# AndreeaPatarlageanu/ConcurrentProject

Hardware: AMD Instinct MI355X
Metric: GCUPS (cell updates/s) for NxN affine-gap SW; bit-exact score vs CPU (higher is better)
Workload: dtype int32; 1 GPU; C2 single pair N=65536 (seed 65536); N=65536, pairs_per_gpu=1, global_pairs=1, parallelism=single GPU, kernel_items=262, blocks=256, boundary_bytes=263207296, W=2, kernel=flow3, half-chunk links, kernel_fn=sw_flow3_kernel, C=32, step=linear-gap identity (G_INIT == G_EXT, exact)

## Files before the change

### concurrentproject_amd/csrc/sw_engine.hip

```cpp
#include "sw_internal.h"
#include "../../include/algoGPU.h"

#include <rccl/rccl.h>
#include <dlfcn.h>

#include <algorithm>
#include <atomic>
#include <chrono>
#include <condition_variable>
#include <functional>
#include <thread>
#include <cstdarg>
#include <cstdio>
#include <cstdlib>
#include <cstring>
#include <map>
#include <mutex>
#include <set>
#include <string>
#include <vector>

namespace swmi {
namespace {

// ... 82 lines not shown
    X(duo_tab, 1, 0, 2, nullptr, false)                                                                               \
                                              \
    X(duo_roles, 1, 0, 1, nullptr, false)                                                                             \
                                         \
    X(duo_raw, 1, 0, 1, nullptr, false)                                                                               \
        \
    X(duo_prio, -1, -1, 20, opt_prio_ok, false)                                                                       \
                                                   \
    X(slab_plain, 0, 0, 1, nullptr, false)                                                                            \
                                                    \
    X(stall_item, -1, -1, ANY_HI, nullptr, false)

#define X(key, def, lo, hi, ok, flag) O_##key,
enum Opt : int { SW_OPTIONS(X) OPT_COUNT };
#undef X
struct OptRow {
    const char* key;
    long long def, lo, hi;
    bool (*ok)(long long);
    bool flag;
};
#define X(key, def, lo, hi, ok, flag) {#key, def, lo, hi, ok, flag},
constexpr OptRow OPT_ROWS[OPT_COUNT] = {SW_OPTIONS(X)};
#undef X
#define X(key, def, lo, hi, ok, flag) {def},
std::atomic<long long> g_opt[OPT_COUNT] = {SW_OPTIONS(X)};
#undef X

struct Opts {
    long long v[OPT_COUNT];
    int f3wedge = -1;
    int f3drops_set = 0;
    int f3drops[4] = {64, 64, 64, 64};
    long long operator[](Opt o) const { return v[o]; }
};
Opts snapshot_opts() {
    Opts o;
    for (int i = 0; i < OPT_COUNT; ++i) o.v[i] = g_opt[i].load();
    const char* w = std::getenv("SWMI_F3WEDGE");
    o.f3wedge = w && w[0] == '0' && !w[1] ? 0 : w && w[0] == '1' && !w[1] ? 1 : -1;
    if (const char* d = std::getenv("SWMI_F3WEDGE_DROPS")) {
        char tail = 0;
        const int got = std::sscanf(d, "%d,%d,%d,%d%c", &o.f3drops[0], &o.f3drops[1], &o.f3drops[2], &o.f3drops[3], &tail);
        o.f3drops_set = got == 4 && wedge_drops_ok(o.f3drops) ? 1 : -1;
    }
    return o;
}
int find_opt(const char* key) {
    for (int i = 0; i < OPT_COUNT; ++i)
        if (std::strcmp(key, OPT_ROWS[i].key) == 0) return i;
    return -1;
}

constexpr long long MAX_SEQ = (1LL << 27) - 1;
constexpr long long RING_AUTO_BYTES = 1LL << 30;

bool want_swap(const Opts& opt, bool single, long long len1, long long len2) {
    const long long o = opt[O_orient];
    if (o == 1) return false;
    if (o == 2) return true;
    return single ? (len2 > len1) : (len1 > len2);
}

bool params_ok(const Params& p) {
    if (p.gap_init < 0 || p.gap_ext < 0 || p.gap_init > (1 << 20) || p.gap_ext > (1 << 20)) {
        set_err("unsupported gap penalties (%d, %d): need 0 <= G_INIT, G_EXT <= 2^20", p.gap_init, p.gap_ext);
        return false;
    }
    if (p.mismatch > 0 || p.mismatch < -127 || p.match > 127 || p.match < p.mismatch) {
        set_err("unsupported scores (MATCH %d, MISMATCH %d): need -127 <= MISMATCH <= 0, MISMATCH <= MATCH <= 127",
                p.match, p.mismatch);
        return false;
    }
// ... 29 lines not shown
        if (p) { HIPCHK(hipHostFree(p)); p = nullptr; cap = 0; }
        size_t want = std::max<size_t>(n, 1);
        want = want + want / 4;
        HIPCHK(hipHostMalloc((void**)&p, want * sizeof(T), hipHostMallocDefault));
        cap = want;
        return 0;
    }
};

struct Ctx {
    int dev = -1;
    int cus = 256;
    hipStream_t own = nullptr;
    hipStream_t last = nullptr;
    hipEvent_t ev0 = nullptr, ev1 = nullptr, staged = nullptr;
    bool staged_pending = false;
    DevBuf<unsigned char> seq;
    DevBuf<PairDesc> desc;
    DevBuf<int> ibase;
    DevBuf<Granule> bnd;
    DevBuf<Ctrl> ctrl;
    DevBuf<int> scores;
    DevBuf<unsigned> flag;
    DevBuf<unsigned> cons;
    DevBuf<unsigned char> hrows;
    DevBuf<DuoDesc> duo;
    PinBuf<DuoDesc> hduo;
    PinBuf<unsigned char> hseq;
    PinBuf<PairDesc> hdesc;
    PinBuf<int> hibase;
    PinBuf<int> hscores;
    PinBuf<Ctrl> hctrl;
    unsigned epoch = 0;
    std::map<int, int> waves_cache;
};

thread_local std::map<int, Ctx*> t_ctx;

Ctx* get_ctx() {
    int dev = 0;
    if (hipGetDevice(&dev) != hipSuccess) {
        set_err("hipGetDevice failed: no HIP device");
        return nullptr;
    }
    auto it = t_ctx.find(dev);
    if (it != t_ctx.end()) return it->second;
    Ctx* c = new Ctx();
    c->dev = dev;
    hipDeviceProp_t prop;
    if (hipGetDeviceProperties(&prop, dev) != hipSuccess) {
        set_err("hipGetDeviceProperties failed");
        delete c;
        return nullptr;
    }
    c->cus = prop.multiProcessorCount;
    if (hipStreamCreateWithFlags(&c->own, hipStreamNonBlocking) != hipSuccess ||
        hipEventCreate(&c->ev0) != hipSuccess || hipEventCreate(&c->ev1) != hipSuccess ||
        hipEventCreateWithFlags(&c->staged, hipEventDisableTiming) != hipSuccess) {
        set_err("stream/event creation failed");
        delete c;
        return nullptr;
    }
    t_ctx[dev] = c;
    return c;
}

// ... 675 lines not shown
    }
    g.wrap_rows = 1;
    while (g.wrap_rows < job.pairs[0].m) g.wrap_rows *= 2;
    job.bnd_granules = (uint64_t)(g.blocks - 1) * (uint64_t)opt[O_ring_rows] + (uint64_t)g.wrap_rows;
    return 0;
}

int size_grid(Ctx* c, Job& job, Variant& v, const Opts& opt, size_t np, Grid& g) {
    const int items = job.item_base[np];
    g.f2_wgs = pick_f2_wgs(job, v, opt, c->cus, items);
    if (v.cfg.duo_wrap > 0) job.bnd_granules = 0;
    if (v.ring && size_ring(job, v, opt, c->cus, items, g)) return -1;
    v.cfg.f2_wgs = g.f2_wgs;
    g.wpc = waves_per_cu(c, v.cfg);
    long long blocks = opt[O_blocks];
    if (blocks <= 0) {
        const int wpb = job.mode == MODE_DUO ? DUO_WAVES : 4;
        const long long cap = (long long)c->cus * std::max(1, g.wpc / wpb);
        const long long want = job.mode == MODE_STRIP ? (items + 3) / 4 : grouped_mode(job.mode) ? items : (long long)np;
        blocks = std::min<long long>(want, cap);
        if (job.mode == MODE_FLOW2) blocks = std::min<long long>(blocks, (long long)c->cus * g.f2_wgs);
    }
    if (v.ring) blocks = g.blocks;
    if (job.f3pwg) {
        blocks = std::min<long long>(np, opt[O_blocks] > 0 ? opt[O_blocks] : (long long)c->cus * g.f2_wgs);
        g.wrap_rows = 64;
        while (g.wrap_rows < v.cfg.max_m) g.wrap_rows *= 2;
        job.bnd_granules = (uint64_t)blocks * (uint64_t)g.wrap_rows;
    }
    v.cfg.blocks = g.blocks = (int)std::max<long long>(1, blocks);
    return 0;
}

int stage_descriptors(Ctx* c, const Job& job, size_t np, hipStream_t s) {
    const bool duo = job.mode == MODE_DUO;
    if (c->staged_pending) {
        HIPCHK(hipEventSynchronize(c->staged));
        c->staged_pending = false;
    }
    if (c->hdesc.ensure(np) || c->hibase.ensure(np + 1) || c->hduo.ensure(np)) return -1;
    if (duo) std::memcpy(c->hduo.p, job.duos.data(), np * sizeof(DuoDesc));
    else std::memcpy(c->hdesc.p, job.pairs.data(), np * sizeof(PairDesc));
    std::memcpy(c->hibase.p, job.item_base.data(), (np + 1) * sizeof(int));
    const Ctrl* ctrl_before = c->ctrl.p;
    if (c->desc.ensure(np, s) || c->duo.ensure(np, s) || c->ibase.ensure(np + 1, s) || c->ctrl.ensure(1, s)) return -1;
    if (c->ctrl.p != ctrl_before) HIPCHK(hipMemsetAsync(c->ctrl.p, 0, sizeof(Ctrl), s));
    return 0;
}

int prepare_device(Ctx* c, const Job& job, const Variant& v, const Opts& opt, const unsigned char* d_seq, int* d_scores,
                   int nscores, size_t np, hipStream_t s) {
    const size_t cons = v.ring ? (size_t)v.cfg.blocks * RING_CONS_STRIDE
                        : v.cfg.duo_wrap > 0 && opt[O_duo_roles] != 0 ? (size_t)DUO_CU_WORDS : 0;
    if (cons) {
        if (c->cons.ensure(cons, s)) return -1;
        HIPCHK(hipMemsetAsync(c->cons.p, 0, cons * sizeof(unsigned), s));
    }
    if (job.bnd_granules) {
        size_t freeb = 0, totb = 0;
        HIPCHK(hipMemGetInfo(&freeb, &totb));
        const size_t need = job.bnd_granules * sizeof(Granule);
        if (need > c->bnd.cap * sizeof(Granule) && need > freeb / 10 * 9) {
            set_err("strip-boundary buffers need %.2f GB, %.2f GB free", need / 1e9, freeb / 1e9);
            return -1;
        }
        if (c->bnd.ensure(job.bnd_granules, s)) return -1;
    }
    if (job.mode == MODE_DUO) HIPCHK(hipMemcpyAsync(c->duo.p, c->hduo.p, np * sizeof(DuoDesc), hipMemcpyHostToDevice, s));
    else HIPCHK(hipMemcpyAsync(c->desc.p, c->hdesc.p, np * sizeof(PairDesc), hipMemcpyHostToDevice, s));
    HIPCHK(hipMemcpyAsync(c->ibase.p, c->hibase.p, (np + 1) * sizeof(int), hipMemcpyHostToDevice, s));
    HIPCHK(hipEventRecord(c->staged, s));
    c->staged_pending = true;
    HIPCHK(hipMemsetAsync(c->ctrl.p, 0, sizeof(unsigned), s));
    HIPCHK(hipMemsetAsync(d_scores, 0, (size_t)nscores * sizeof(int), s));
    if (v.cfg.hep && v.ring) {
        const PairDesc& d = job.pairs[0];
        if (c->hrows.ensure((size_t)d.m, s)) return -1;
        HepSel t{};
        for (int b = 0; b < 256; ++b) {
            const unsigned sym = job.hsym[b];
            t.sel[b] = (unsigned char)(sym < 4 ? 4 + sym : sym - 3);
        }
        hipLaunchKernelGGL(hep_rows_kernel, dim3((unsigned)std::min(1024, (d.m + 255) / 256)), dim3(256), 0, s,
                           d_seq + d.row_off, d.m, c->hrows.p, t);
        HIPCHK(hipGetLastError());
    }
    return 0;
}

void fill_score_words(KParams& kp, const Params& prm, const unsigned char* hsym) {
    kp.match = prm.match;
    kp.mismatch = prm.mismatch;
    kp.gap_init = prm.gap_init;
    kp.gap_ext = prm.gap_ext;
    profile_words(prm, kp.prof);
    for (int q = 0; q < 4; ++q) {
        unsigned w2 = 0, w3 = 0, pen = 0;
        for (int r = 0; r < 4; ++r) {
            const int sc = r == q ? prm.match : prm.mismatch;
            w2 |= (unsigned)((sc + prm.gap_init) & 0xFF) << (8 * r);
            w3 |= (unsigned)(sc & 0xFF) << (8 * r);
            pen |= (unsigned)(prm.match - sc) << (8 * r);
        }
        kp.prof2[q] = w2;
        kp.prof3[q] = w3;
        kp.pen[q] = pen;
    }
    if (!hsym) return;
    std::memcpy(kp.hsym, hsym, sizeof kp.hsym);
    for (int c = 0; c < 7; ++c) {
        unsigned p2 = 0, q2 = 0x80u, p3 = 0, q3 = 0x80u;
        for (int r = 0; r < 7; ++r) {
            const int sc = r == c ? prm.match : prm.mismatch;
            const unsigned b2 = (unsigned)((sc + prm.gap_init) & 0xFF), b3 = (unsigned)(sc & 0xFF);
            if (r < 4) {
                p2 |= b2 << (8 * r);
                p3 |= b3 << (8 * r);
            } else {
                q2 |= b2 << (8 * (r - 3));
                q3 |= b3 << (8 * (r - 3));
            }
        }
        kp.hp2[c] = p2;
        kp.hq2[c] = q2;
        kp.hp3[c] = p3;
        kp.hq3[c] = q3;
    }
}

KParams fill_kparams(Ctx* c, const Job& job, const Variant& v, const Grid& g, const Params& prm, const Opts& opt,
                     const unsigned char* d_seq, int* d_scores, size_t np, const SlabEdge* edge) {
    KParams kp{};
    kp.seq = d_seq;
    kp.pairs = c->desc.p;
    kp.duos = c->duo.p;
    kp.item_base = c->ibase.p;
    kp.bnd = c->bnd.p;
    kp.ctrl = c->ctrl.p;
    kp.scores = d_scores;
    kp.npairs = (int)np;
    kp.total_items = job.item_base[np];
    do ++c->epoch;
    while (c->epoch == 0 || ((c->epoch ^ 0x5BD1E995u) & 31u) == 0 || ((c->epoch ^ 0x5BD1E995u ^ 0x9E3779B9u) & 31u) == 0);
    kp.epoch = c->epoch;
    fill_score_words(kp, prm, v.cfg.hep ? job.hsym : nullptr);
    if (v.cfg.duo_wrap > 0) {
        kp.wrap_rows = v.cfg.duo_wrap;
        if (opt[O_duo_roles] != 0) kp.ring_cons = c->cons.p;
        const int dp = (int)opt[O_duo_prio];
        kp.duo_prio = dp >= 0 ? dp : v.cfg.duo_tab > 0 ? 17 : 0;
    }
    kp.timeout_ticks = opt[O_timeout] * 100000000LL;
    kp.stall_item = (int)opt[O_stall_item];
    kp.w45_s4 = v.cfg.f3_w45 ? job.w45_s4 : -1;
    kp.trace = reinterpret_cast<unsigned long long*>(opt[O_trace]);
    if (v.ring) {
        kp.ring_rows = (int)opt[O_ring_rows];
        kp.wrap_rows = g.wrap_rows;
        kp.ring_cons = c->cons.p;
    }
    if (job.f3pwg) kp.wrap_rows = g.wrap_rows;
    if (v.wedge) {
        kp.wedge = 1;
        kp.wedge_e0[0] = job.wplan.e0[0];
        kp.wedge_e0[1] = job.wplan.e0[1];
        kp.wedge_rlead = job.wplan.rlead;
        kp.wedge_rows = job.wedge_rows;
        kp.wedge_bnd[0] = job.wedge_bnd[0];
        kp.wedge_bnd[1] = job.wedge_bnd[1];
        for (int j = 0; j < 4; ++j) kp.wedge_drop[j] = job.wplan.drop[j];
        kp.wedge_segr = job.wedge_segr;
        kp.wedge_seg[0] = job.wedge_seg[0];
        kp.wedge_seg[1] = job.wedge_seg[1];
    }
    if (v.cfg.hep && v.ring) kp.hrows = c->hrows.p;
    if (edge) {
        kp.slab_in = edge->in;
        kp.slab_out = edge->out;
        kp.slab_epoch = edge->epoch;
    }
    return kp;
}

int enqueue(Ctx* c, Job& job, const Params& prm, const Opts& opt, const unsigned char* d_seq, int* d_scores, int nscores,
            hipStream_t s, bool time_kernel, const SlabEdge* edge = nullptr) {
    if (job.mode == MODE_FLOW2 ? !flow2_variant_exists(job.C) : !variant_exists(job.W, job.C)) {
        set_err("no kernel variant for W=%d C=%d", job.W, job.C);
        return -1;
    }
    if (opt.f3drops_set < 0) {
        set_err("SWMI_F3WEDGE_DROPS: need d0,d1,d2,d3, multiples of 64 from 64 to %d with d0 == d2", WEDGE_DROP_MAX);
        return -1;
    }
    if (!plan_wedge(job, prm, opt, c->cus)) plan_split(job, prm, opt, c->cus);
    Variant v = select_variant(job, prm, opt, c->cus);
    if (v.err) {
        set_err("%s", v.err);
        return -1;
    }
    const size_t np = job.mode == MODE_DUO ? job.duos.size() : job.pairs.size();
    Grid g;
    if (stage_descriptors(c, job, np, s) || size_grid(c, job, v, opt, np, g) ||
        prepare_device(c, job, v, opt, d_seq, d_scores, nscores, np, s))
        return -1;
    const KParams kp = fill_kparams(c, job, v, g, prm, opt, d_seq, d_scores, np, edge);

    if (time_kernel) HIPCHK(hipEventRecord(c->ev0, s));
    HIPCHK(v.cfg.f3 || v.cfg.f3a || v.cfg.f3ra ? launch_sw_flow3(v.cfg, kp, s)
           : job.mode == MODE_FLOW2           ? launch_sw_flow2(v.cfg, kp, s) : launch_sw_strip(v.cfg, kp, s));
    if (v.cut) {
        const PairDesc& l = job.pairs[0];
        const PairDesc& r = job.pairs[1];
        const Granule* gl = c->bnd.p + l.bnd_off + (uint64_t)((l.strips + 3) / 4 - 1) * (uint64_t)l.m;
        const Granule* gr = c->bnd.p + r.bnd_off + (uint64_t)((r.strips + 3) / 4 - 1) * (uint64_t)r.m;
        HIPCHK(launch_sw_flow3_combine(gl, gr, l.m, prm.gap_init, kp.epoch, c->ctrl.p, d_scores + l.out_idx, s));
    }
    if (v.steep) {
        const SteepJoin j = {c->bnd.p + job.wedge_bnd[0], c->bnd.p + job.wedge_bnd[1], c->bnd.p + job.pairs[0].bnd_off,
                             c->bnd.p + job.pairs[1].bnd_off, c->bnd.p + job.wedge_seg[0], c->bnd.p + job.wedge_seg[1],
                             job.wedge_rows, job.wedge_segr, job.pairs[0].m, prm.gap_init};
        HIPCHK(launch_sw_flow3_steep_combine(j, job.wplan, kp.epoch, c->ctrl.p, d_scores + job.pairs[0].out_idx, s));
    } else if (v.wedge)
        HIPCHK(launch_sw_flow3_wedge_combine(c->bnd.p + job.wedge_bnd[0], c->bnd.p + job.wedge_bnd[1], job.wplan,
                                             job.pairs[0].m, kp.epoch, c->ctrl.p, d_scores + job.pairs[0].out_idx, s));
    if (time_kernel) HIPCHK(hipEventRecord(c->ev1, s));

    t_stats = sw_stats{};
    t_stats.cells = job.cells;
    t_stats.W = job.W;
    t_stats.C = job.C;
    t_stats.dna = job.hep ? 2 : job.dna ? 1 : 0;
    t_stats.blocks = v.cfg.blocks;
    t_stats.waves_per_cu = g.wpc;
    t_stats.items = job.item_base[np];
    t_stats.mode = job.mode;
    t_stats.variant = variant_word(v);
    t_stats.boundary_bytes = (long long)(job.bnd_granules * sizeof(Granule));
    c->last = s;
    return 0;
}

int check_ctrl(Ctx* c, hipStream_t s) {
    if (c->hctrl.ensure(1)) return -1;
    HIPCHK(hipMemcpyAsync(c->hctrl.p, c->ctrl.p, sizeof(Ctrl), hipMemcpyDeviceToHost, s));
    HIPCHK(hipStreamSynchronize(s));
    if (c->hctrl.p->error) {
        if (c->hctrl.p->error == ERR_EDGE)
            set_err("a cut pair's final edge held a row that this launch never wrote (error %u)", c->hctrl.p->error);
        else
            set_err("strip hand-off timed out (error %u, strip %u): a producer strip never published",
                    c->hctrl.p->error, c->hctrl.p->err_item);
        HIPCHK(hipMemsetAsync(c->ctrl.p, 0, sizeof(Ctrl), s));
        HIPCHK(hipStreamSynchronize(s));
        return -1;
    }
    return 0;
}

struct HostPair {
    const unsigned char* s1;
    int n;
    const unsigned char* s2;
    int m;
};

int check_host_pairs(const HostPair* in, int npairs, const Params& prm) {
    if (npairs < 0 || (npairs > 0 && !in)) {
        set_err("invalid arguments");
        return -1;
    }
    if (!params_ok(prm)) return -1;
    for (int k = 0; k < npairs; ++k) {
        if (in[k].n < 0 || in[k].m < 0 || (in[k].n > 0 && !in[k].s1) || (in[k].m > 0 && !in[k].s2)) {
            set_err("pair %d: invalid sequence pointer/length", k);
            return -1;
        }
        if ((long long)std::min(in[k].n, in[k].m) * std::max(prm.match, 1) >= (1LL << 28)) {
            set_err("pair %d: score range exceeds the int32 engine (min length * MATCH >= 2^28)", k);
            return -1;
        }
        if (in[k].n > MAX_SEQ || in[k].m > MAX_SEQ) {
            set_err("pair %d: sequences longer than 2^27 - 1 bytes are not supported", k);
            return -1;
        }
    }
// ... 779 lines not shown
```

### concurrentproject_amd/csrc/sw_flow3.hip

```cpp
#include <algorithm>
#include <type_traits>

#include "sw_device.h"

namespace swmi {
namespace {

typedef unsigned int u32x2 __attribute__((ext_vector_type(2)));

constexpr int F3_R = 512;
constexpr int F3_RS = 2 * F3_R + 64;
constexpr int F3_BIG = 0x3FFFFFFF;
constexpr int F3_THREADS = 320;
constexpr unsigned F3_KEY = 0x5BD1E995u;
enum : int { F3_NONE = 0, F3_LDS = 1, F3_GRAN = 2, F3_PEER = 3 };

__device__ __forceinline__ unsigned lds_addr(const void* p) {
    return (unsigned)(uintptr_t)(const __attribute__((address_space(3))) void*)p;
}

struct F3Loop {
    int pA, pB;
    int ng;
    int G;
// ... 42 lines not shown

struct F3PLoop {
    int pA, pB;
    int ng, nge;
    int G, GE;
    unsigned k80;
    unsigned code;
    unsigned lin;
    unsigned lout;
    unsigned lrb;
    unsigned pin, pout, qme, qnx;
    int end;
    unsigned dlo, dhi;
    __amdgpu_buffer_rsrc_t rsrc;
    unsigned ek, ek2;
    int lrow;
    unsigned long long m16;
    unsigned long long l63;
    unsigned lsc;
};
template <int AFF, int IN, int OUT, int SH>
__device__ F3Res f3p_loop(const F3PLoop& x);

#include "sw_flow3p_loops.inc"

constexpr unsigned F3_KEY2 = 0x9E3779B9u;
__device__ __forceinline__ unsigned f3_slab_key(unsigned epoch) { return (epoch << 5) ^ (F3_KEY & ~31u) ^ 0x15u; }

__host__ __device__ constexpr int f3_chunks(int m, int C) { return (((m + 64 + C - 1) / C) + 1) & ~1; }
constexpr int F3P_PAD = 16;
__host__ __device__ constexpr int f3_stage_bytes(int m, int C) { return (64 + (f3_chunks(m, C) + 4) * C + 64 + 15) & ~15; }
constexpr int f3_static_lds(bool aff) { return 5 * F3_RS * (aff ? 8 : 4) + 64; }

template <int C, int HL, bool AFF, bool POOL = false, bool HEP = false>
__device__ __forceinline__ void flow3_staged(const KParams& kp) {
    static_assert(!POOL || C == 32, "pool loops run 32-row chunks");
    static_assert(!(POOL && HEP), "seven-letter alphabets run the rotating loops");
    using Slot = typename std::conditional<AFF, int2, int>::type;
    constexpr int H = HL ? C / 2 : C;
    extern __shared__ __attribute__((aligned(16))) unsigned char rc[];
    __shared__ __attribute__((aligned(16))) Slot ring[5][F3_RS];
    __shared__ int prod[5], cons[5];
    __shared__ int s_item;
    const int tid = threadIdx.x;
    const int lane = tid & 63;
    const int wave = __builtin_amdgcn_readfirstlane((int)(tid >> 6));
    const int go = kp.gap_init, ge = kp.gap_ext;
    Slot init;
    if constexpr (AFF) init = make_int2(-go, -ge);
    else init = -go;
    for (;;) {
        if (tid == 0) s_item = (int)atomicAdd(&kp.ctrl->next_item, 1u);
        __syncthreads();
        const int item = __builtin_amdgcn_readfirstlane(s_item);
        if (item >= kp.total_items) return;
        const bool wedge = !AFF && !POOL && kp.wedge != 0;
        const int pi = wedge ? (item & 1) : find_pair(kp, item);
        const PairDesc pd = load_pair(kp, pi);
        const int m = pd.m;
        const int group = wedge ? (item >> 1) : item - kp.item_base[pi];
        const int ngroups = (pd.strips + 3) / 4;
        const int chunks = f3_chunks(m + (POOL ? F3P_PAD : 0), C);
        const int w_end =
            wedge ? kp.wedge_e0[pi] - (kp.wedge_drop[0] + kp.wedge_drop[1] + kp.wedge_drop[2] + kp.wedge_drop[3]) * group : 0;
        const int w_cum = !wedge || wave == 0 || wave > 3 ? 0
                          : kp.wedge_drop[0] + (wave > 1 ? kp.wedge_drop[1] : 0) + (wave > 2 ? kp.wedge_drop[2] : 0);
        const int rl = wedge && (pd.flags & PAIR_REV) != 0 ? kp.wedge_rlead : 0;
        const int mt = m + rl;
        const auto edge_of = [&](int b) {
            if (!wedge) return group_edge(kp, pd, b, ngroups);
            return linear_edge(kp.bnd + pd.bnd_off + (uint64_t)b * (uint64_t)kp.wedge_rows, kp.wedge_rows, kp.epoch);
        };
        if (tid < 5) {
            prod[tid] = POOL ? -64 : -H;
            cons[tid] = F3_R;
        }
        for (int i = tid; i < 5 * F3_RS; i += F3_THREADS) (&ring[0][0])[i] = init;
        const __amdgpu_buffer_rsrc_t row_rsrc =
            __builtin_amdgcn_make_buffer_rsrc(const_cast<unsigned char*>(kp.seq + pd.row_off), 0, m, RSRC_FLAGS);
        const int nst = wedge ? (64 + w_end + 4 * C + 64 + 15) & ~15 : f3_stage_bytes(m + (POOL ? F3P_PAD : 0), C);
        const bool rev = !AFF && !POOL && (pd.flags & PAIR_REV) != 0;
        const bool rev16 = rev && (((unsigned)pd.row_off + (unsigned)mt) & 3u) == 0u;
        for (int i = tid * 16; i < nst; i += 16 * F3_THREADS) {
            const int row0 = i - 64;
            u32x4 w = u32x4{0u, 0u, 0u, 0u};
            if constexpr (HEP) {
#pragma unroll
                for (int j = 0; j < 16; ++j) {
                    const int row = row0 + j;
                    const bool live = row >= rl && row < mt;
                    const unsigned ch = __builtin_amdgcn_raw_buffer_load_b8(
// ... 191 lines not shown
            } else {
                x.pA = (int)(liveA ? kp.prof2[dna_code(kp.seq[offA])] : 0x80808080u);
                x.pB = (int)(liveB ? kp.prof3[dna_code(kp.seq[offB])] : 0x80808080u);
            }
            x.ng = -go;
            x.G = go;
            x.code = lds_addr(rc) + 64u - (unsigned)lane;
            x.lin = lds_addr(&ring[in_ring][0]) + 4u * (unsigned)(64 + C + (lane & (C - 1)));
            x.lout = lds_addr(&ring[wave][0]) + 4u * (unsigned)((lane + C) & 63);
            x.pin = lds_addr(&prod[in_ring]);
            x.pout = lds_addr(&prod[wave]);
            x.qme = lds_addr(&cons[in_ring]);
            x.qnx = lds_addr(&cons[wave]);
            x.end = wedge ? w_end - w_cum : chunks * C;
            x.dlo = (unsigned)dl;
            x.dhi = (unsigned)(dl >> 32);
            x.rsrc = edge_of(group).rsrc;
            x.ek = kp.epoch ^ F3_KEY;
            x.lrow = (lane - 128) * 8;
            x.m48 = ~0ull << (64 - C / 2);
            x.lmid = 4u * (16u + (lane >= 32 && lane < 48 ? 32u : 0u));
            if (in_kind == F3_LDS) {
                r = out_kind == F3_LDS ? f3_loop<C, HL, F3_LDS, F3_LDS>(x)
                    : out_kind == F3_GRAN ? f3_loop<C, HL, F3_LDS, F3_GRAN>(x)
                                          : f3_loop<C, HL, F3_LDS, F3_NONE>(x);
            } else {
                r = out_kind == F3_LDS ? f3_loop<C, HL, F3_NONE, F3_LDS>(x)
                    : out_kind == F3_GRAN ? f3_loop<C, HL, F3_NONE, F3_GRAN>(x)
                                          : f3_loop<C, HL, F3_NONE, F3_NONE>(x);
            }
            if (wedge) {
                u32x4* wb = reinterpret_cast<u32x4*>(kp.bnd + kp.wedge_bnd[pi]) + 2 * (64 * strip + lane);
                const unsigned ek = kp.epoch ^ F3_KEY;
                wb[0] = u32x4{(unsigned)r.a0, (unsigned)r.b0, (unsigned)r.a0 ^ ek, (unsigned)r.b0 ^ ek};
                wb[1] = u32x4{(unsigned)r.a1, (unsigned)r.b1, (unsigned)r.a1 ^ ek, (unsigned)r.b1 ^ ek};
                if (kp.wedge_segr > 0 && out_kind != F3_NONE) {
                    const int drop = kp.wedge_drop[wave & 3];
                    u32x2* sg = reinterpret_cast<u32x2*>(kp.bnd + kp.wedge_seg[pi]) + (uint64_t)strip * (uint64_t)kp.wedge_segr;
                    if (lane == 63) sg[0] = u32x2{(unsigned)r.io, (unsigned)r.io ^ ek};
                    if (out_kind == F3_LDS) {
                        for (int k = lane; k < drop - 63; k += 64) {
                            const int v = ring[wave][((x.end - drop - 1 + k + 128) & (F3_R - 1)) + F3_R];
                            sg[1 + k] = u32x2{(unsigned)v, (unsigned)v ^ ek};
                        }
                    }
                }
            }
        }
        if (kp.trace != nullptr && lane == 0) {
            unsigned long long* t = kp.trace + 16ull * (unsigned)strip;
            t[0] = (unsigned long long)t_start;
            t[1] = (unsigned long long)t_start;
            t[3] = (unsigned long long)r.slow;
            t[2] = (unsigned long long)__builtin_amdgcn_s_memrealtime();
            t[4] = (unsigned)__builtin_amdgcn_s_getreg((31 << 11) | 4);
            t[5] = (unsigned)__builtin_amdgcn_s_getreg((31 << 11) | 20);
            t[7] = (unsigned long long)chunks;
        }
        if (r.fail && lane == 0) {
            atomicOr(&kp.ctrl->error, ERR_TIMEOUT);
            atomicMax(&kp.ctrl->err_item, (unsigned)strip);
        }
        int M = r.M;
#pragma unroll
        for (int off = 32; off > 0; off >>= 1) M = max(M, __shfl_xor(M, off));
        if (lane == 0 && M > 0) atomicMax(&kp.scores[pd.out_idx], M);
    }
}

template <int C, int HL>
__global__ void __launch_bounds__(F3_THREADS) sw_flow3_kernel(KParams kp) {
    flow3_staged<C, HL, false>(kp);
}
template <int C, int HL>
__global__ void __launch_bounds__(F3_THREADS) sw_flow3a_kernel(KParams kp) {
    flow3_staged<C, HL, true>(kp);
}
template <int C, int HL>
__global__ void __launch_bounds__(F3_THREADS) sw_flow3h_kernel(KParams kp) {
    flow3_staged<C, HL, false, false, true>(kp);
}
template <int C, int HL>
__global__ void __launch_bounds__(F3_THREADS) sw_flow3ah_kernel(KParams kp) {
    flow3_staged<C, HL, true, false, true>(kp);
}
template <int AFF>
__global__ void __launch_bounds__(F3_THREADS) sw_flow3p_kernel(KParams kp) {
    flow3_staged<32, 1, AFF != 0, true>(kp);
}

constexpr int F3_COMBINE_THREADS = 256;
__global__ void __launch_bounds__(F3_COMBINE_THREADS)
sw_flow3_combine_kernel(const u32x2* __restrict__ gl, const u32x2* __restrict__ gr, int m, int g2, unsigned ek,
                        Ctrl* ctrl, int* score) {
    int best = 0;
    bool bad = false;
// ... 22 lines not shown
        const int s = idx >> 6, l = idx & 63;
        const int c = 126 * s + 2 * l, W = 126 * S + 2;
        const int i0 = e0f - 64 * s - l;
        u32x4 f[2] = {bf[2 * idx], bf[2 * idx + 1]};
        bad |= (f[0].z != (f[0].x ^ ek)) | (f[0].w != (f[0].y ^ ek)) | (f[1].z != (f[1].x ^ ek)) | (f[1].w != (f[1].y ^ ek));
        for (int col = 0; col < 2; ++col) {
            const int p = W - 2 - c - 2 * col;
            if (p < 0) continue;
            const int sp = p / 126, lp = (p % 126) >> 1;
            for (int dup = 0; dup < 2; ++dup) {
                const int s2 = sp - dup, l2 = dup ? 63 : lp;
                if (s2 < 0 || s2 >= S || (dup && lp != 0)) continue;
                const int r = m - 1 + rlead - (e0b - 64 * s2 - 1 - l2);
                const u32x4 g[2] = {bb[2 * (64 * s2 + l2)], bb[2 * (64 * s2 + l2) + 1]};
                bad |= (g[0].z != (g[0].x ^ ek)) | (g[0].w != (g[0].y ^ ek)) | (g[1].z != (g[1].x ^ ek)) |
                       (g[1].w != (g[1].y ^ ek));
                for (int k = 0; k < (l == 0 && s > 0 ? 1 : 2); ++k)
                    for (int k2 = 0; k2 < (l2 == 0 && s2 > 0 ? 1 : 2); ++k2)
                        if (i0 + k == r - k2)
                            best = max(best, (int)(col ? f[k].y : f[k].x) + (int)(col ? g[k2].y : g[k2].x));
            }
        }
    }
    if (bad) best = 0;
#pragma unroll
    for (int off = 32; off > 0; off >>= 1) best = max(best, __shfl_xor(best, off));
    const bool any_bad = __ballot(bad) != 0ull;
    if ((threadIdx.x & 63) == 0) {
        if (best > 0) atomicMax(score, best);
        if (any_bad) atomicOr(&ctrl->error, ERR_EDGE);
    }
}

struct SteepArgs {
    const u32x4 *bf, *bb;
    const u32x2 *ef, *eb, *sf, *sb;
    int S, m, e0f, e0b, rlead, edge_rows, segr, maxcol, gap;
    int drop[4];
    unsigned ek;
};
__device__ __forceinline__ int steep_cum_dev(const SteepArgs& a, int s) {
    int c = (s >> 2) * (a.drop[0] + a.drop[1] + a.drop[2] + a.drop[3]);
    if ((s & 3) > 0) c += a.drop[0];
    if ((s & 3) > 1) c += a.drop[1];
    if ((s & 3) > 2) c += a.drop[2];
    return c;
}
__device__ __forceinline__ int steep_col_h(const SteepArgs& a, const u32x4* lanes, const u32x2* edge, const u32x2* seg,
                                           int s, int end, int drop, int t, bool& bad) {
    if (t >= drop - 62) {
        const u32x4 e = lanes[2 * (64 * s + 62) + (t - (drop - 62))];
        bad |= e.w != (e.y ^ a.ek);
        return (int)e.y;
    }
    const u32x2 g = t == drop - 63   ? seg[(size_t)s * (size_t)a.segr]
                    : (s & 3) == 3 ? edge[(size_t)(s >> 2) * 2u * (size_t)a.edge_rows + (size_t)(end - drop - 1 + t)]
                                   : seg[(size_t)s * (size_t)a.segr + 1u + (size_t)t];
    bad |= g.y != (g.x ^ a.ek);
    return (int)g.x + a.gap;
}
__global__ void __launch_bounds__(F3_COMBINE_THREADS)
sw_flow3_steep_combine_kernel(SteepArgs a, Ctrl* ctrl, int* score) {
    int best = 0;
    bool bad = false;
    const int S = a.S;
    const unsigned ek = a.ek;
    const int idx = (int)(blockIdx.x * F3_COMBINE_THREADS + threadIdx.x);
    if (idx < 64 * S) {
        const int s = idx >> 6, l = idx & 63;
        const int c = 126 * s + 2 * l, W = 126 * S + 2;
        const int i0 = a.e0f - steep_cum_dev(a, s) - l;
        u32x4 f[2] = {a.bf[2 * idx], a.bf[2 * idx + 1]};
        bad |= (f[0].z != (f[0].x ^ ek)) | (f[0].w != (f[0].y ^ ek)) | (f[1].z != (f[1].x ^ ek)) | (f[1].w != (f[1].y ^ ek));
        for (int col = 0; col < 2; ++col) {
            const int p = W - 4 - c - 2 * col;
            if (p < 0) continue;
            const int sp = p / 126, lp = (p % 126) >> 1;
            for (int dup = 0; dup < 2; ++dup) {
                const int s2 = sp - dup, l2 = dup ? 63 : lp;
                if (s2 < 0 || s2 >= S || (dup && lp != 0)) continue;
                const int r = a.m - 1 + a.rlead - (a.e0b - steep_cum_dev(a, s2) - 1 - l2);
                const u32x4 g[2] = {a.bb[2 * (64 * s2 + l2)], a.bb[2 * (64 * s2 + l2) + 1]};
                bad |= (g[0].z != (g[0].x ^ ek)) | (g[0].w != (g[0].y ^ ek)) | (g[1].z != (g[1].x ^ ek)) |
                       (g[1].w != (g[1].y ^ ek));
                for (int k = 0; k < (l == 0 && s > 0 ? 1 : 2); ++k)
                    for (int k2 = 0; k2 < (l2 == 0 && s2 > 0 ? 1 : 2); ++k2)
                        if (i0 + k == r - k2)
                            best = max(best, (int)(col ? f[k].y : f[k].x) + (int)(col ? g[k2].y : g[k2].x));
            }
        }
    } else if (idx - 64 * S < (S - 1) * a.maxcol) {
        const int s = (idx - 64 * S) / a.maxcol, k = (idx - 64 * S) % a.maxcol;
        const int drop = a.drop[s & 3];
        if (k < drop - 60) {
            const int s2 = S - 2 - s;
            const int endf = a.e0f - steep_cum_dev(a, s), endb = a.e0b - steep_cum_dev(a, s2);
            const int i = endf - drop + k;
            const int kb = a.m - 1 + a.rlead - i - (endb - drop - 1);
            if (kb >= 0 && kb <= drop - 61) {
                const int hf = steep_col_h(a, a.bf, a.ef, a.sf, s, endf, drop, k, bad);
                const int hb = steep_col_h(a, a.bb, a.eb, a.sb, s2, endb, drop, kb, bad);
                best = max(best, hf + hb);
            } else {
                bad = true;
            }
        }
    }
    if (bad) best = 0;
#pragma unroll
    for (int off = 32; off > 0; off >>= 1) best = max(best, __shfl_xor(best, off));
    const bool any_bad = __ballot(bad) != 0ull;
    if ((threadIdx.x & 63) == 0) {
        if (best > 0) atomicMax(score, best);
        if (any_bad) atomicOr(&ctrl->error, ERR_EDGE);
    }
}

#ifndef SW_F3R_R
#define SW_F3R_R 512
#endif
constexpr int F3R_R = SW_F3R_R;
constexpr int F3R_RS = F3R_R + 64;
constexpr int F3R_THREADS = 256;
constexpr int F3R_CRB = 384;
__host__ __device__ constexpr int f3r_chunks(int m, int C) { return (((m + 64 + C - 1) / C) + 1) & ~1; }

struct F3RLoop {
    int pA, pB, ng, G;
    int pC;
    int pD, pE;
    unsigned k80;
    unsigned qA, qB, qC;
    int m, end;
    unsigned dlo, dhi;
    int lane;
    unsigned raw2;
    unsigned cro;
    unsigned c0, cbase;
    unsigned cwr, cwm;
// ... 617 lines not shown
```

### concurrentproject_amd/csrc/sw_internal.h

```cpp
#pragma once
#include <hip/hip_runtime.h>
#include <stdint.h>

#include <algorithm>

namespace swmi {

struct PairDesc {
    uint64_t col_off;
    uint64_t row_off;
    uint64_t bnd_off;
    int n;
    int m;
    int strips;
    int out_idx;
    int flags;
    int lead;
};
enum : int { PAIR_HALF = 1, PAIR_REV = 2, PAIR_WEDGE = 4 };

struct DuoDesc {
    uint64_t col_off[2];
    uint64_t row_off[2];
    uint64_t bnd_off;
// ... 32 lines not shown
    Ctrl* ctrl;
    int* scores;
    int npairs;
    int total_items;
    unsigned epoch;
    int match, mismatch, gap_init, gap_ext;
    unsigned prof[4];
    unsigned prof2[4];
    unsigned prof3[4];
    unsigned pen[4];
    unsigned char hsym[256];
    unsigned hp2[7], hq2[7], hp3[7], hq3[7];
    const unsigned char* hrows;
    const DuoDesc* duos;
    long long timeout_ticks;
    unsigned long long* trace;
    Granule* slab_in;
    Granule* slab_out;
    unsigned slab_epoch;
    int ring_rows;
    int wrap_rows;
    unsigned* ring_cons;
    int duo_prio;
    int w45_s4;
    int stall_item;
    int wedge;
    int wedge_e0[2];
    int wedge_rlead;
    int wedge_rows;
    unsigned long long wedge_bnd[2];
    int wedge_drop[4];
    int wedge_segr;
    unsigned long long wedge_seg[2];
};

constexpr int RING_CONS_STRIDE = 32;

enum : int { MODE_STRIP = 0, MODE_PAIRWG = 1, MODE_CHAIN = 2, MODE_DUO = 3, MODE_FLOW = 4, MODE_FLOW2 = 5 };
inline bool grouped_mode(int mode) { return mode == MODE_CHAIN || mode == MODE_FLOW || mode == MODE_FLOW2; }

#ifndef SW_DUO_WAVES
#define SW_DUO_WAVES 4
#endif
constexpr int DUO_WAVES = SW_DUO_WAVES;

struct LaunchCfg {
    int W;
    int C;
    bool dna;
    int blocks;
    int mode;
    int max_m;
    bool duo_f16 = false;
    bool f2_stream = false;
    int f2_wgs = 1;
    bool f2_lin = false;
    bool f2_w2 = false;
    bool f2_pwg = false;
    bool f3 = false;
    bool f3_hl = false;
    bool f3a = false;
    bool f3p = false;
    bool hep = false;
    bool f3_w3 = false;
    bool f3_w45 = false;
    bool f3_pwg = false;
    bool f3ra = false;
// ... 118 lines not shown
```

Baseline: 3285 GCUPS.

## Fuse wedge join into flow3 kernel and skip per-call descriptor staging

```diff
diff --git a/concurrentproject_amd/csrc/sw_engine.hip b/concurrentproject_amd/csrc/sw_engine.hip
--- a/concurrentproject_amd/csrc/sw_engine.hip
+++ b/concurrentproject_amd/csrc/sw_engine.hip
@@ -138,6 +138,7 @@
     int f3wedge = -1;
     int f3drops_set = 0;
     int f3drops[4] = {64, 64, 64, 64};
+    int f3join = 1;
     long long operator[](Opt o) const { return v[o]; }
 };
 Opts snapshot_opts() {
@@ -145,6 +146,8 @@
     for (int i = 0; i < OPT_COUNT; ++i) o.v[i] = g_opt[i].load();
     const char* w = std::getenv("SWMI_F3WEDGE");
     o.f3wedge = w && w[0] == '0' && !w[1] ? 0 : w && w[0] == '1' && !w[1] ? 1 : -1;
+    const char* j = std::getenv("SWMI_F3JOIN");
+    o.f3join = j && j[0] == '0' && !j[1] ? 0 : 1;
     if (const char* d = std::getenv("SWMI_F3WEDGE_DROPS")) {
         char tail = 0;
         const int got = std::sscanf(d, "%d,%d,%d,%d%c", &o.f3drops[0], &o.f3drops[1], &o.f3drops[2], &o.f3drops[3], &tail);
@@ -240,6 +243,9 @@
     PinBuf<int> hscores;
     PinBuf<Ctrl> hctrl;
     unsigned epoch = 0;
+    DevBuf<unsigned> join;
+    unsigned item0 = 0;
+    bool item0_known = false;
     std::map<int, int> waves_cache;
 };
 
@@ -981,8 +987,25 @@
     return 0;
 }
 
-int stage_descriptors(Ctx* c, const Job& job, size_t np, hipStream_t s) {
+int stage_descriptors(Ctx* c, const Job& job, size_t np, bool join, hipStream_t s) {
     const bool duo = job.mode == MODE_DUO;
+    const Ctrl* ctrl_before = c->ctrl.p;
+    if (join) {
+        const size_t join_before = c->join.cap;
+        const size_t words = (size_t)JOIN_UNITS + (size_t)job.wplan.strips;
+        if (c->ctrl.ensure(1, s) || c->join.ensure(words, s)) return -1;
+        if (c->ctrl.p != ctrl_before) {
+            HIPCHK(hipMemsetAsync(c->ctrl.p, 0, sizeof(Ctrl), s));
+            c->item0 = 0;
+            c->item0_known = true;
+        } else if (!c->item0_known) {
+            HIPCHK(hipMemsetAsync(c->ctrl.p, 0, sizeof(unsigned), s));
+            c->item0 = 0;
+            c->item0_known = true;
+        }
+        if (c->join.cap != join_before) HIPCHK(hipMemsetAsync(c->join.p, 0, c->join.cap * sizeof(unsigned), s));
+        return 0;
+    }
     if (c->staged_pending) {
         HIPCHK(hipEventSynchronize(c->staged));
         c->staged_pending = false;
@@ -991,14 +1014,13 @@
     if (duo) std::memcpy(c->hduo.p, job.duos.data(), np * sizeof(DuoDesc));
     else std::memcpy(c->hdesc.p, job.pairs.data(), np * sizeof(PairDesc));
     std::memcpy(c->hibase.p, job.item_base.data(), (np + 1) * sizeof(int));
-    const Ctrl* ctrl_before = c->ctrl.p;
     if (c->desc.ensure(np, s) || c->duo.ensure(np, s) || c->ibase.ensure(np + 1, s) || c->ctrl.ensure(1, s)) return -1;
     if (c->ctrl.p != ctrl_before) HIPCHK(hipMemsetAsync(c->ctrl.p, 0, sizeof(Ctrl), s));
     return 0;
 }
 
 int prepare_device(Ctx* c, const Job& job, const Variant& v, const Opts& opt, const unsigned char* d_seq, int* d_scores,
-                   int nscores, size_t np, hipStream_t s) {
+                   int nscores, size_t np, bool join, hipStream_t s) {
     const size_t cons = v.ring ? (size_t)v.cfg.blocks * RING_CONS_STRIDE
                         : v.cfg.duo_wrap > 0 && opt[O_duo_roles] != 0 ? (size_t)DUO_CU_WORDS : 0;
     if (cons) {
@@ -1015,12 +1037,17 @@
         }
         if (c->bnd.ensure(job.bnd_granules, s)) return -1;
     }
+    if (join) {
+        if (nscores > 1) HIPCHK(hipMemsetAsync(d_scores, 0, (size_t)nscores * sizeof(int), s));
+        return 0;
+    }
     if (job.mode == MODE_DUO) HIPCHK(hipMemcpyAsync(c->duo.p, c->hduo.p, np * sizeof(DuoDesc), hipMemcpyHostToDevice, s));
     else HIPCHK(hipMemcpyAsync(c->desc.p, c->hdesc.p, np * sizeof(PairDesc), hipMemcpyHostToDevice, s));
     HIPCHK(hipMemcpyAsync(c->ibase.p, c->hibase.p, (np + 1) * sizeof(int), hipMemcpyHostToDevice, s));
     HIPCHK(hipEventRecord(c->staged, s));
     c->staged_pending = true;
     HIPCHK(hipMemsetAsync(c->ctrl.p, 0, sizeof(unsigned), s));
+    c->item0_known = false;
     HIPCHK(hipMemsetAsync(d_scores, 0, (size_t)nscores * sizeof(int), s));
     if (v.cfg.hep && v.ring) {
         const PairDesc& d = job.pairs[0];
@@ -1078,7 +1105,8 @@
 }
 
 KParams fill_kparams(Ctx* c, const Job& job, const Variant& v, const Grid& g, const Params& prm, const Opts& opt,
-                     const unsigned char* d_seq, int* d_scores, size_t np, const SlabEdge* edge) {
+                     const unsigned char* d_seq, int* d_scores, size_t np, const SlabEdge* edge, bool join, hipStream_t s,
+                     int* err) {
     KParams kp{};
     kp.seq = d_seq;
     kp.pairs = c->desc.p;
@@ -1089,9 +1117,13 @@
     kp.scores = d_scores;
     kp.npairs = (int)np;
     kp.total_items = job.item_base[np];
+    const unsigned epoch_before = c->epoch;
     do ++c->epoch;
     while (c->epoch == 0 || ((c->epoch ^ 0x5BD1E995u) & 31u) == 0 || ((c->epoch ^ 0x5BD1E995u ^ 0x9E3779B9u) & 31u) == 0);
     kp.epoch = c->epoch;
+    if (c->epoch < epoch_before && c->join.p &&
+        hipMemsetAsync(c->join.p + JOIN_SCORE, 0, 2 * sizeof(unsigned), s) != hipSuccess)
+        *err = -1;
     fill_score_words(kp, prm, v.cfg.hep ? job.hsym : nullptr);
     if (v.cfg.duo_wrap > 0) {
         kp.wrap_rows = v.cfg.duo_wrap;
@@ -1121,6 +1153,12 @@
         kp.wedge_segr = job.wedge_segr;
         kp.wedge_seg[0] = job.wedge_seg[0];
         kp.wedge_seg[1] = job.wedge_seg[1];
+        if (join) {
+            kp.wedge_join = c->join.p;
+            kp.item0 = c->item0;
+            kp.wedge_pair[0] = job.pairs[0];
+            kp.wedge_pair[1] = job.pairs[1];
+        }
     }
     if (v.cfg.hep && v.ring) kp.hrows = c->hrows.p;
     if (edge) {
@@ -1149,10 +1187,16 @@
     }
     const size_t np = job.mode == MODE_DUO ? job.duos.size() : job.pairs.size();
     Grid g;
-    if (stage_descriptors(c, job, np, s) || size_grid(c, job, v, opt, np, g) ||
-        prepare_device(c, job, v, opt, d_seq, d_scores, nscores, np, s))
-        return -1;
-    const KParams kp = fill_kparams(c, job, v, g, prm, opt, d_seq, d_scores, np, edge);
+    const bool join = v.wedge && opt.f3join != 0;
+    if (stage_descriptors(c, job, np, join, s) || size_grid(c, job, v, opt, np, g) ||
+        prepare_device(c, job, v, opt, d_seq, d_scores, nscores, np, join, s))
+        return -1;
+    int kerr = 0;
+    const KParams kp = fill_kparams(c, job, v, g, prm, opt, d_seq, d_scores, np, edge, join, s, &kerr);
+    if (kerr) {
+        set_err("clearing the join words failed");
+        return -1;
+    }
 
     if (time_kernel) HIPCHK(hipEventRecord(c->ev0, s));
     HIPCHK(v.cfg.f3 || v.cfg.f3a || v.cfg.f3ra ? launch_sw_flow3(v.cfg, kp, s)
@@ -1164,7 +1208,9 @@
         const Granule* gr = c->bnd.p + r.bnd_off + (uint64_t)((r.strips + 3) / 4 - 1) * (uint64_t)r.m;
         HIPCHK(launch_sw_flow3_combine(gl, gr, l.m, prm.gap_init, kp.epoch, c->ctrl.p, d_scores + l.out_idx, s));
     }
-    if (v.steep) {
+    if (join) {
+        c->item0 += (unsigned)kp.total_items + (unsigned)v.cfg.blocks;
+    } else if (v.steep) {
         const SteepJoin j = {c->bnd.p + job.wedge_bnd[0], c->bnd.p + job.wedge_bnd[1], c->bnd.p + job.pairs[0].bnd_off,
                              c->bnd.p + job.pairs[1].bnd_off, c->bnd.p + job.wedge_seg[0], c->bnd.p + job.wedge_seg[1],
                              job.wedge_rows, job.wedge_segr, job.pairs[0].m, prm.gap_init};
@@ -1200,6 +1246,9 @@
             set_err("strip hand-off timed out (error %u, strip %u): a producer strip never published",
                     c->hctrl.p->error, c->hctrl.p->err_item);
         HIPCHK(hipMemsetAsync(c->ctrl.p, 0, sizeof(Ctrl), s));
+        c->item0 = 0;
+        c->item0_known = true;
+        if (c->join.p) HIPCHK(hipMemsetAsync(c->join.p, 0, c->join.cap * sizeof(unsigned), s));
         HIPCHK(hipStreamSynchronize(s));
         return -1;
     }
diff --git a/concurrentproject_amd/csrc/sw_flow3.hip b/concurrentproject_amd/csrc/sw_flow3.hip
--- a/concurrentproject_amd/csrc/sw_flow3.hip
+++ b/concurrentproject_amd/csrc/sw_flow3.hip
@@ -98,6 +98,177 @@
 __host__ __device__ constexpr int f3_stage_bytes(int m, int C) { return (64 + (f3_chunks(m, C) + 4) * C + 64 + 15) & ~15; }
 constexpr int f3_static_lds(bool aff) { return 5 * F3_RS * (aff ? 8 : 4) + 64; }
 
+struct SteepArgs {
+    const u32x4 *bf, *bb;
+    const u32x2 *ef, *eb, *sf, *sb;
+    int S, m, e0f, e0b, rlead, edge_rows, segr, maxcol, gap;
+    int drop[4];
+    unsigned ek;
+    int pshift = 4;
+};
+template <bool SC1>
+__device__ __forceinline__ u32x2 join_ld8(const u32x2* p) {
+    if constexpr (SC1) {
+        const unsigned long long v = __hip_atomic_load(reinterpret_cast<unsigned long long*>(const_cast<u32x2*>(p)),
+                                                       __ATOMIC_RELAXED, __HIP_MEMORY_SCOPE_AGENT);
+        return u32x2{(unsigned)v, (unsigned)(v >> 32)};
+    } else {
+        return *p;
+    }
+}
+__device__ __forceinline__ void join_st8(u32x2* p, unsigned lo, unsigned hi) {
+    __hip_atomic_store(reinterpret_cast<unsigned long long*>(p), (unsigned long long)lo | ((unsigned long long)hi << 32),
+                       __ATOMIC_RELAXED, __HIP_MEMORY_SCOPE_AGENT);
+}
+__device__ __forceinline__ void join_drain() {
+    compiler_fence();
+    __builtin_amdgcn_s_waitcnt(0);
+    compiler_fence();
+}
+template <bool SC1>
+__device__ __forceinline__ u32x4 join_ld16(const u32x4* p) {
+    if constexpr (SC1) {
+        const u32x2 lo = join_ld8<true>(reinterpret_cast<const u32x2*>(p));
+        const u32x2 hi = join_ld8<true>(reinterpret_cast<const u32x2*>(p) + 1);
+        return u32x4{lo.x, lo.y, hi.x, hi.y};
+    } else {
+        return *p;
+    }
+}
+__device__ __forceinline__ int steep_cum_dev(const SteepArgs& a, int s) {
+    int c = (s >> 2) * (a.drop[0] + a.drop[1] + a.drop[2] + a.drop[3]);
+    if ((s & 3) > 0) c += a.drop[0];
+    if ((s & 3) > 1) c += a.drop[1];
+    if ((s & 3) > 2) c += a.drop[2];
+    return c;
+}
+__device__ __forceinline__ int steep_drop_dev(const SteepArgs& a, int s) {
+    const int j = s & 3;
+    return j == 0 ? a.drop[0] : j == 1 ? a.drop[1] : j == 2 ? a.drop[2] : a.drop[3];
+}
+template <bool SC1>
+__device__ __forceinline__ int steep_col_h(const SteepArgs& a, const u32x4* lanes, const u32x2* edge, const u32x2* seg,
+                                           int s, int end, int drop, int t, bool& bad) {
+    if (t >= drop - 62) {
+        const u32x4 e = join_ld16<SC1>(lanes + 2 * (64 * s + 62) + (t - (drop - 62)));
+        bad |= e.w != (e.y ^ a.ek);
+        return (int)e.y;
+    }
+    const u32x2 g = join_ld8<SC1>(t == drop - 63 ? seg + (size_t)s * (size_t)a.segr
+                                  : (s & 3) == 3 ? edge + (size_t)(s >> 2) * 2u * (size_t)a.edge_rows + (size_t)(end - drop - 1 + t)
+                                                 : seg + (size_t)s * (size_t)a.segr + 1u + (size_t)t);
+    bad |= g.y != (g.x ^ a.ek);
+    return (int)g.x + a.gap;
+}
+template <bool SC1>
+__device__ __forceinline__ void join_diag(const SteepArgs& a, int s, int l, int& best, bool& bad) {
+    const int S = a.S;
+    const unsigned ek = a.ek;
+    const int idx = 64 * s + l;
+    const int c = 126 * s + 2 * l, W = 126 * S + 2;
+    const int i0 = a.e0f - steep_cum_dev(a, s) - l;
+    const u32x4 f[2] = {join_ld16<SC1>(a.bf + 2 * idx), join_ld16<SC1>(a.bf + 2 * idx + 1)};
+    bad |= (f[0].z != (f[0].x ^ ek)) | (f[0].w != (f[0].y ^ ek)) | (f[1].z != (f[1].x ^ ek)) | (f[1].w != (f[1].y ^ ek));
+    for (int col = 0; col < 2; ++col) {
+        const int p = W - a.pshift - c - 2 * col;
+        if (p < 0) continue;
+        const int sp = p / 126, lp = (p % 126) >> 1;
+        for (int dup = 0; dup < 2; ++dup) {
+            const int s2 = sp - dup, l2 = dup ? 63 : lp;
+            if (s2 < 0 || s2 >= S || (dup && lp != 0)) continue;
+            const int r = a.m - 1 + a.rlead - (a.e0b - steep_cum_dev(a, s2) - 1 - l2);
+            const u32x4 g[2] = {join_ld16<SC1>(a.bb + 2 * (64 * s2 + l2)), join_ld16<SC1>(a.bb + 2 * (64 * s2 + l2) + 1)};
+            bad |= (g[0].z != (g[0].x ^ ek)) | (g[0].w != (g[0].y ^ ek)) | (g[1].z != (g[1].x ^ ek)) |
+                   (g[1].w != (g[1].y ^ ek));
+            for (int k = 0; k < (l == 0 && s > 0 ? 1 : 2); ++k)
+                for (int k2 = 0; k2 < (l2 == 0 && s2 > 0 ? 1 : 2); ++k2)
+                    if (i0 + k == r - k2)
+                        best = max(best, (int)(col ? f[k].y : f[k].x) + (int)(col ? g[k2].y : g[k2].x));
+        }
+    }
+}
+template <bool SC1>
+__device__ __forceinline__ void join_col(const SteepArgs& a, int s, int k, int& best, bool& bad) {
+    const int S = a.S;
+    const int drop = steep_drop_dev(a, s);
+    if (k < drop - 60) {
+        const int s2 = S - 2 - s;
+        const int endf = a.e0f - steep_cum_dev(a, s), endb = a.e0b - steep_cum_dev(a, s2);
+        const int i = endf - drop + k;
+        const int kb = a.m - 1 + a.rlead - i - (endb - drop - 1);
+        if (kb >= 0 && kb <= drop - 61) {
+            const int hf = steep_col_h<SC1>(a, a.bf, a.ef, a.sf, s, endf, drop, k, bad);
+            const int hb = steep_col_h<SC1>(a, a.bb, a.eb, a.sb, s2, endb, drop, kb, bad);
+            best = max(best, hf + hb);
+        } else {
+            bad = true;
+        }
+    }
+}
+
+__device__ __forceinline__ void f3_join_strip(const KParams& kp, const PairDesc& pd, int pi, int strip, int M, int lane) {
+    const int S = pd.strips;
+    const bool steep = kp.wedge_segr > 0;
+    unsigned* jw = kp.wedge_join;
+    const int u0 = pi == 0 ? strip : max(S - strip - 2, 0);
+    const int u1 = pi == 0 ? strip : min(S - strip - (steep ? 1 : 0), S - 1);
+    M = max(M, 0);
+    join_drain();
+    bool won = false;
+    if (lane <= u1 - u0) won = (int)atomicAdd(&jw[JOIN_UNITS + u0 + lane], 1u) + 1 == join_unit_full(S, u0 + lane, steep);
+    unsigned long long wins = __ballot(won);
+    while (wins != 0ull) {
+        const int u = u0 + (int)__builtin_ctzll(wins);
+        wins &= wins - 1ull;
+        SteepArgs a;
+        a.bf = reinterpret_cast<const u32x4*>(kp.bnd + kp.wedge_bnd[0]);
+        a.bb = reinterpret_cast<const u32x4*>(kp.bnd + kp.wedge_bnd[1]);
+        a.ef = reinterpret_cast<const u32x2*>(kp.bnd + kp.wedge_pair[0].bnd_off);
+        a.eb = reinterpret_cast<const u32x2*>(kp.bnd + kp.wedge_pair[1].bnd_off);
+        a.sf = reinterpret_cast<const u32x2*>(kp.bnd + kp.wedge_seg[0]);
+        a.sb = reinterpret_cast<const u32x2*>(kp.bnd + kp.wedge_seg[1]);
+        a.S = S;
+        a.m = pd.m;
+        a.e0f = kp.wedge_e0[0];
+        a.e0b = kp.wedge_e0[1];
+        a.rlead = kp.wedge_rlead;
+        a.edge_rows = kp.wedge_rows;
+        a.segr = kp.wedge_segr;
+        a.maxcol = max(max(kp.wedge_drop[0], kp.wedge_drop[1]), max(kp.wedge_drop[2], kp.wedge_drop[3])) - 60;
+        a.gap = kp.gap_init;
+        a.drop[0] = kp.wedge_drop[0];
+        a.drop[1] = kp.wedge_drop[1];
+        a.drop[2] = kp.wedge_drop[2];
+        a.drop[3] = kp.wedge_drop[3];
+        a.ek = kp.epoch ^ F3_KEY;
+        a.pshift = steep ? 4 : 2;
+        int best = 0;
+        bool bad = false;
+        join_diag<true>(a, u, lane, best, bad);
+        if (steep && u < S - 1)
+            for (int k = lane; k < a.maxcol; k += 64) join_col<true>(a, u, k, best, bad);
+        if (bad) best = 0;
+        M = max(M, best);
+        const bool any_bad = __ballot(bad) != 0ull;
+        if (lane == 0) {
+            __hip_atomic_store(&jw[JOIN_UNITS + u], 0u, __ATOMIC_RELAXED, __HIP_MEMORY_SCOPE_AGENT);
+            if (any_bad) atomicOr(&kp.ctrl->error, ERR_EDGE);
+        }
+    }
+#pragma unroll
+    for (int off = 32; off > 0; off >>= 1) M = max(M, __shfl_xor(M, off));
+    if (lane == 0) {
+        unsigned long long* word = reinterpret_cast<unsigned long long*>(jw + JOIN_SCORE);
+        atomicMax(word, ((unsigned long long)kp.epoch << 32) | (unsigned long long)(unsigned)M);
+        join_drain();
+        if (atomicAdd(&jw[JOIN_DONE], 1u) + 1u == 2u * (unsigned)S) {
+            const unsigned long long v = atomicMax(word, 0ull);
+            kp.scores[pd.out_idx] = (int)(unsigned)v;
+            __hip_atomic_store(&jw[JOIN_DONE], 0u, __ATOMIC_RELAXED, __HIP_MEMORY_SCOPE_AGENT);
+        }
+    }
+}
+
 template <int C, int HL, bool AFF, bool POOL = false, bool HEP = false>
 __device__ __forceinline__ void flow3_staged(const KParams& kp) {
     static_assert(!POOL || C == 32, "pool loops run 32-row chunks");
@@ -116,13 +287,14 @@
     if constexpr (AFF) init = make_int2(-go, -ge);
     else init = -go;
     for (;;) {
-        if (tid == 0) s_item = (int)atomicAdd(&kp.ctrl->next_item, 1u);
+        if (tid == 0) s_item = (int)(atomicAdd(&kp.ctrl->next_item, 1u) - kp.item0);
         __syncthreads();
         const int item = __builtin_amdgcn_readfirstlane(s_item);
         if (item >= kp.total_items) return;
         const bool wedge = !AFF && !POOL && kp.wedge != 0;
         const int pi = wedge ? (item & 1) : find_pair(kp, item);
-        const PairDesc pd = load_pair(kp, pi);
+        const bool join = wedge && kp.wedge_join != nullptr;
+        const PairDesc pd = join ? (pi ? kp.wedge_pair[1] : kp.wedge_pair[0]) : load_pair(kp, pi);
         const int m = pd.m;
         const int group = wedge ? (item >> 1) : item - kp.item_base[pi];
         const int ngroups = (pd.strips + 3) / 4;
@@ -380,16 +552,28 @@
             if (wedge) {
                 u32x4* wb = reinterpret_cast<u32x4*>(kp.bnd + kp.wedge_bnd[pi]) + 2 * (64 * strip + lane);
                 const unsigned ek = kp.epoch ^ F3_KEY;
-                wb[0] = u32x4{(unsigned)r.a0, (unsigned)r.b0, (unsigned)r.a0 ^ ek, (unsigned)r.b0 ^ ek};
-                wb[1] = u32x4{(unsigned)r.a1, (unsigned)r.b1, (unsigned)r.a1 ^ ek, (unsigned)r.b1 ^ ek};
+                if (join) {
+                    u32x2* w2 = reinterpret_cast<u32x2*>(wb);
+                    join_st8(w2 + 0, (unsigned)r.a0, (unsigned)r.b0);
+                    join_st8(w2 + 1, (unsigned)r.a0 ^ ek, (unsigned)r.b0 ^ ek);
+                    join_st8(w2 + 2, (unsigned)r.a1, (unsigned)r.b1);
+                    join_st8(w2 + 3, (unsigned)r.a1 ^ ek, (unsigned)r.b1 ^ ek);
+                } else {
+                    wb[0] = u32x4{(unsigned)r.a0, (unsigned)r.b0, (unsigned)r.a0 ^ ek, (unsigned)r.b0 ^ ek};
+                    wb[1] = u32x4{(unsigned)r.a1, (unsigned)r.b1, (unsigned)r.a1 ^ ek, (unsigned)r.b1 ^ ek};
+                }
                 if (kp.wedge_segr > 0 && out_kind != F3_NONE) {
                     const int drop = kp.wedge_drop[wave & 3];
                     u32x2* sg = reinterpret_cast<u32x2*>(kp.bnd + kp.wedge_seg[pi]) + (uint64_t)strip * (uint64_t)kp.wedge_segr;
-                    if (lane == 63) sg[0] = u32x2{(unsigned)r.io, (unsigned)r.io ^ ek};
+                    if (lane == 63) {
+                        if (join) join_st8(sg, (unsigned)r.io, (unsigned)r.io ^ ek);
+                        else sg[0] = u32x2{(unsigned)r.io, (unsigned)r.io ^ ek};
+                    }
                     if (out_kind == F3_LDS) {
                         for (int k = lane; k < drop - 63; k += 64) {
                             const int v = ring[wave][((x.end - drop - 1 + k + 128) & (F3_R - 1)) + F3_R];
-                            sg[1 + k] = u32x2{(unsigned)v, (unsigned)v ^ ek};
+                            if (join) join_st8(sg + 1 + k, (unsigned)v, (unsigned)v ^ ek);
+                            else sg[1 + k] = u32x2{(unsigned)v, (unsigned)v ^ ek};
                         }
                     }
                 }
@@ -410,6 +594,12 @@
             atomicMax(&kp.ctrl->err_item, (unsigned)strip);
         }
         int M = r.M;
+        if constexpr (!AFF && !POOL) {
+            if (join) {
+                f3_join_strip(kp, pd, pi, strip, M, lane);
+                continue;
+            }
+        }
 #pragma unroll
         for (int off = 32; off > 0; off >>= 1) M = max(M, __shfl_xor(M, off));
         if (lane == 0 && M > 0) atomicMax(&kp.scores[pd.out_idx], M);
@@ -498,79 +688,16 @@
     }
 }
 
-struct SteepArgs {
-    const u32x4 *bf, *bb;
-    const u32x2 *ef, *eb, *sf, *sb;
-    int S, m, e0f, e0b, rlead, edge_rows, segr, maxcol, gap;
-    int drop[4];
-    unsigned ek;
-};
-__device__ __forceinline__ int steep_cum_dev(const SteepArgs& a, int s) {
-    int c = (s >> 2) * (a.drop[0] + a.drop[1] + a.drop[2] + a.drop[3]);
-    if ((s & 3) > 0) c += a.drop[0];
-    if ((s & 3) > 1) c += a.drop[1];
-    if ((s & 3) > 2) c += a.drop[2];
-    return c;
-}
-__device__ __forceinline__ int steep_col_h(const SteepArgs& a, const u32x4* lanes, const u32x2* edge, const u32x2* seg,
-                                           int s, int end, int drop, int t, bool& bad) {
-    if (t >= drop - 62) {
-        const u32x4 e = lanes[2 * (64 * s + 62) + (t - (drop - 62))];
-        bad |= e.w != (e.y ^ a.ek);
-        return (int)e.y;
-    }
-    const u32x2 g = t == drop - 63   ? seg[(size_t)s * (size_t)a.segr]
-                    : (s & 3) == 3 ? edge[(size_t)(s >> 2) * 2u * (size_t)a.edge_rows + (size_t)(end - drop - 1 + t)]
-                                   : seg[(size_t)s * (size_t)a.segr + 1u + (size_t)t];
-    bad |= g.y != (g.x ^ a.ek);
-    return (int)g.x + a.gap;
-}
 __global__ void __launch_bounds__(F3_COMBINE_THREADS)
 sw_flow3_steep_combine_kernel(SteepArgs a, Ctrl* ctrl, int* score) {
     int best = 0;
     bool bad = false;
     const int S = a.S;
-    const unsigned ek = a.ek;
     const int idx = (int)(blockIdx.x * F3_COMBINE_THREADS + threadIdx.x);
     if (idx < 64 * S) {
-        const int s = idx >> 6, l = idx & 63;
-        const int c = 126 * s + 2 * l, W = 126 * S + 2;
-        const int i0 = a.e0f - steep_cum_dev(a, s) - l;
-        u32x4 f[2] = {a.bf[2 * idx], a.bf[2 * idx + 1]};
-        bad |= (f[0].z != (f[0].x ^ ek)) | (f[0].w != (f[0].y ^ ek)) | (f[1].z != (f[1].x ^ ek)) | (f[1].w != (f[1].y ^ ek));
-        for (int col = 0; col < 2; ++col) {
-            const int p = W - 4 - c - 2 * col;
-            if (p < 0) continue;
-            const int sp = p / 126, lp = (p % 126) >> 1;
-            for (int dup = 0; dup < 2; ++dup) {
-                const int s2 = sp - dup, l2 = dup ? 63 : lp;
-                if (s2 < 0 || s2 >= S || (dup && lp != 0)) continue;
-                const int r = a.m - 1 + a.rlead - (a.e0b - steep_cum_dev(a, s2) - 1 - l2);
-                const u32x4 g[2] = {a.bb[2 * (64 * s2 + l2)], a.bb[2 * (64 * s2 + l2) + 1]};
-                bad |= (g[0].z != (g[0].x ^ ek)) | (g[0].w != (g[0].y ^ ek)) | (g[1].z != (g[1].x ^ ek)) |
-                       (g[1].w != (g[1].y ^ ek));
-                for (int k = 0; k < (l == 0 && s > 0 ? 1 : 2); ++k)
-                    for (int k2 = 0; k2 < (l2 == 0 && s2 > 0 ? 1 : 2); ++k2)
-                        if (i0 + k == r - k2)
-                            best = max(best, (int)(col ? f[k].y : f[k].x) + (int)(col ? g[k2].y : g[k2].x));
-            }
-        }
+        join_diag<false>(a, idx >> 6, idx & 63, best, bad);
     } else if (idx - 64 * S < (S - 1) * a.maxcol) {
-        const int s = (idx - 64 * S) / a.maxcol, k = (idx - 64 * S) % a.maxcol;
-        const int drop = a.drop[s & 3];
-        if (k < drop - 60) {
-            const int s2 = S - 2 - s;
-            const int endf = a.e0f - steep_cum_dev(a, s), endb = a.e0b - steep_cum_dev(a, s2);
-            const int i = endf - drop + k;
-            const int kb = a.m - 1 + a.rlead - i - (endb - drop - 1);
-            if (kb >= 0 && kb <= drop - 61) {
-                const int hf = steep_col_h(a, a.bf, a.ef, a.sf, s, endf, drop, k, bad);
-                const int hb = steep_col_h(a, a.bb, a.eb, a.sb, s2, endb, drop, kb, bad);
-                best = max(best, hf + hb);
-            } else {
-                bad = true;
-            }
-        }
+        join_col<false>(a, (idx - 64 * S) / a.maxcol, (idx - 64 * S) % a.maxcol, best, bad);
     }
     if (bad) best = 0;
 #pragma unroll
diff --git a/concurrentproject_amd/csrc/sw_internal.h b/concurrentproject_amd/csrc/sw_internal.h
--- a/concurrentproject_amd/csrc/sw_internal.h
+++ b/concurrentproject_amd/csrc/sw_internal.h
@@ -88,7 +88,19 @@
     int wedge_drop[4];
     int wedge_segr;
     unsigned long long wedge_seg[2];
-};
+    unsigned* wedge_join;
+    unsigned item0;
+    PairDesc wedge_pair[2];
+};
+enum : int { JOIN_SCORE = 0, JOIN_DONE = 2, JOIN_UNITS = 4 };
+__host__ __device__ inline int join_unit_lo(int S, int s, bool steep) { return S - s - 2 < 0 ? 0 : S - s - 2; }
+__host__ __device__ inline int join_unit_hi(int S, int s, bool steep) {
+    const int hi = S - s - (steep ? 1 : 0);
+    return hi > S - 1 ? S - 1 : hi;
+}
+__host__ __device__ inline int join_unit_full(int S, int s, bool steep) {
+    return 1 + join_unit_hi(S, s, steep) - join_unit_lo(S, s, steep) + 1;
+}
 
 constexpr int RING_CONS_STRIDE = 32;
 
```

After: 3343 GCUPS, median of 6. 1.02x the previous value.
